# jacobwulffwold/GAN_SR_wind_field

Hardware: AMD Instinct MI355X
Metric: GAN train-steps/sec (G+D fwd+bwd) (higher is better)
Workload: dtype bf16; 1 GPU; C3' full G+D adversarial step: LR 32x32x128 -> HR 128x128x128 (x4), batch 1/GPU, G 16 RRDB nf128 (34.77M), D bf32; preset=C3p, global_batch=1, parallelism=dp1, ranks=1

## Files before the change

### gan_sr_wind_field_amd/csrc/conv_tile.hip

```cpp
#include <cstdlib>

#include "conv_tile_impl.h"

int wsr_ct_run_n144(CtArgs& a, int tpk, hipStream_t st);
int wsr_ct_run_n128(CtArgs& a, int tpk, hipStream_t st);
int wsr_ct_run_narrow(CtArgs& a, int tpk, hipStream_t st);
int wsr_ct_run_wide(CtArgs& a, int tpk, hipStream_t st);
int wsr_ct_run_masked(CtArgs& a, int tpk, hipStream_t st);
int wsr_ct_run_narrow_masked(CtArgs& a, int tpk, hipStream_t st);
int wsr_ct_run_small(CtArgs& a, int tpk, hipStream_t st);
int wsr_ct_run_tm3(CtArgs& a, int tpk, hipStream_t st);
int wsr_ct_run_simple_narrow(CtArgs& a, int tpk, int tm3, hipStream_t st);
int wsr_ct_run_simple_n128(CtArgs& a, int tpk, int tm3, hipStream_t st);
int wsr_ct_run_simple_small(CtArgs& a, int tpk, hipStream_t st);
long wsr_ct_tiles(const CtArgs& a, int rows);
int wsr_ct_run_strided(CtArgs& a, int tpk, hipStream_t st);
int wsr_ct_run_f32(CtArgs& a, int tpk, hipStream_t st);

namespace {

int dispatch_ct(CtArgs& a, int tpk, hipStream_t st) {
  const int N = a.Cout;
  if (a.f32) return wsr_ct_run_f32(a, tpk, st);
  if ((a.sx | a.sy | a.sz) != 1) return wsr_ct_run_strided(a, tpk, st);
// ... 450 lines not shown
  a.alpha = 1.f;
  if (ep) {
    a.bias = ep->bias;
    a.chan_scale = ep->chan_scale;
    a.res = (const unsigned short*)ep->res;
    a.res_ctot = ep->res_ctot;
    a.res_off = ep->res_off;
    a.res_c1 = 0x7FFFFFFF;
    a.alpha = ep->alpha;
    a.beta = ep->beta;
    a.slope = ep->slope;
    a.act = ep->act;
    a.act_c1 = ep->act_c1 > 0 ? ep->act_c1 : 0x7FFFFFFF;
    if (a.act == 2 && (!a.res || ep->out_planar)) return WSR_EINVAL;
    a.out_planar = ep->out_planar;
    if (a.res && (a.res_off < 0 || a.res_off + c->Cout > a.res_ctot)) return WSR_EINVAL;
    a.ws = ep->ws;
    a.ws_bytes = (long)ep->ws_bytes;
    if (two) {
      a.in2 = (const unsigned short*)ep->in2;
      a.in2_ctot = ep->in2_ctot;
      a.in2_chunk = ep->in2_c0;
    }
    if (ep->mask) {
      const wsr_lrelu_mask_t* mk = ep->mask;
      if (!mk->y || ep->out_planar || mk->c0 < 0 || mk->c1 > c->Cout || mk->c0 >= mk->c1 || mk->c0 % 4 || mk->y_ctot % 4 ||
          mk->y_off % 4 || mk->y_off + (mk->c1 - mk->c0) > mk->y_ctot || mk->chan_scale)
        return WSR_EINVAL;
      if (f32) return WSR_EUNSUPPORTED;
      a.mask_y = (const unsigned short*)mk->y;
      a.mask_ctot = mk->y_ctot; a.mask_off = mk->y_off;
      a.mask_c0 = mk->c0; a.mask_c1 = mk->c1;
      a.mask_slope = mk->slope;
    }
  }
  a.B = c->B; a.Xi = c->Xi; a.Yi = c->Yi; a.Zi = c->Zi;
  a.Xo = c->Xo; a.Yo = c->Yo; a.Zo = c->Zo;
  a.ups = c->upsample_xy ? 1 : 0;
  a.in_ctot = c->in_ctot; a.in_off = c->in_off;
  a.Cout = c->Cout; a.out_ctot = c->out_ctot; a.out_off = c->out_off;
  a.KX = c->KX; a.KY = c->KY; a.KZ = c->KZ;
  a.px = c->px; a.py = c->py; a.pz = c->pz;
  if (c->lat) {
    if (a.res || a.out_planar) return WSR_EUNSUPPORTED;
    a.ol_m = 2; a.ol_ox = c->lat_ox; a.ol_oy = c->lat_oy;
    a.ol_mz = c->lat_mz > 1 ? c->lat_mz : 1; a.ol_oz = c->lat_oz;
    a.nphase = c->lat_phases == 4 ? 4 : 1;
    a.ph_wstride = (long)wsr_frag_filter_elems(c->Cout, c->Cin, c->KX * c->KY * c->KZ, c->dtype);
  }
  if (f32 && c->KX * c->KY * c->KZ == 1) return WSR_EUNSUPPORTED;
  if (!f32 && !a.mask_y && c->KX * c->KY * c->KZ == 1 && !c->lat && !a.ups && !a.out_planar && !a.chan_scale && (c->px | c->py | c->pz) == 0 &&
      (c->sx | c->sy | c->sz) == 1 && a.act <= 1 && a.act_c1 == 0x7FFFFFFF) {
    const int rc = wsr_conv1x1_bf16(a.in, a.in_ctot, a.in_off, c->Cin, a.wf, (unsigned short*)a.out, a.out_ctot,
                                    a.out_off, a.Cout, (long)c->B * c->Xo * c->Yo * c->Zo, a.bias, a.res, a.res_ctot,
                                    a.res_off, a.res ? a.res_c1 : 0, a.alpha, a.beta, a.act, a.slope, nullptr,
                                    ep ? (const unsigned short*)ep->res2 : nullptr, ep ? ep->res2_ctot : 0,
                                    ep ? ep->res2_off : 0, ep ? ep->beta2 : 0.f, as_stream(stream));
    if (rc != WSR_EUNSUPPORTED) return rc;
  }
  if (ep && ep->res2) return WSR_EUNSUPPORTED;
  if (two) return run_conv_tile(a, c->Cin, as_stream(stream));
  const bool no_slide = WSR_ENV_SET("WSR_NO_SLIDE");
  if (!f32 && !no_slide && c->KZ == 1 && c->Cout <= 16 && a.out_planar && !a.chan_scale && !a.res && a.act == 0 && !a.ups &&
      !c->lat && (c->sx | c->sy | c->sz) == 1 && c->pz == 0 && a.alpha == 1.f && c->Xo == c->Xi && c->Yo == c->Yi &&
      zero_page()) {
    const int rc = wsr_conv_slide_fwd(a.in, a.in_ctot, a.in_off, c->Cin, a.wf, (float*)a.out, c->Cout, c->B, c->Xi, c->Yi,
// ... 107 lines not shown
```

### gan_sr_wind_field_amd/csrc/conv_tile_impl.h

```cpp
#pragma once
#include <cstdlib>
#include <type_traits>

#include "common.h"

struct CtArgs {
  const unsigned short* in;
  const unsigned short* wf;
  void* out;
  const void* zero16;
  const float* bias;
  const float* chan_scale;
  const unsigned short* res;
  int res_ctot, res_off, res_c1;
  float alpha, beta, slope;
  int act, out_planar;
  int act_c1;
  int B, Xi, Yi, Zi, Xo, Yo, Zo, ups;
  int in_ctot, in_off, nchunks;
  int cin_valid;
  int Cout, out_ctot, out_off;
  int KX, KY, KZ, px, py, pz;
  int sx, sy, sz;
  int TX, TY, TZ;
  int tiles_x, tiles_y, tiles_z, ntiles;
  int nts;
  int TS;
  int NT_total;
  int ngroups;
  int P;
  int off_mtab, off_htab, off_ttab, off_btab, off_xs, off_ws;
  int vec_ok;
  const unsigned short* mask_y;
  int mask_ctot, mask_off, mask_c0, mask_c1;
  float mask_slope;
  int xbufs;
  unsigned mg_TZ, mg_TY, mg_Lz, mg_Ly, mg_KZ, mg_KY, mg_ng, mg_tz, mg_ty, mg_tx;
  int il_m, il_ox, il_oy, ol_m, ol_ox, ol_oy, nphase;
  int ol_mz, ol_oz;
  long ph_wstride;
  int ksplit, cps;
  float* part;
  long part_stride;
  void* ws;
  long ws_bytes;
  int xs_stage, xs_units;
  const unsigned short* in2;
  int in2_ctot, in2_chunk;
  void* out2;
  int out2_ctot, out2_c0;
  int f32;
  int prio;
  int ablate;
  unsigned long long* stamps;
};

int wsr_ct_splitk_reduce(const CtArgs& a, hipStream_t st);

void wsr_ct_note_plan(const CtArgs& a, int ntw);
void wsr_ct_note_inst(int wm, int wn, int tm, int tn, int tpk, int mask, int f32, int wk, int simple);

namespace {

__device__ __forceinline__ void glds16(const void* gsrc, unsigned lds_addr) {
  unsigned keep;
  asm volatile(
      "s_mov_b32 %0, m0\n\ts_mov_b32 m0, %2\n\ts_nop 0\n\tglobal_load_lds_dwordx4 %1, off\n\ts_mov_b32 m0, %0"
      : "=&s"(keep)
      : "v"(gsrc), "s"(lds_addr)
      : "memory");
}
__device__ __forceinline__ void dma_wait() { asm volatile("s_waitcnt vmcnt(0)" ::: "memory"); }

#ifdef WSR_CT_STAMPS
#define CT_STAMP(k)                                                                                   \
  do {                                                                                                \
    if (a.stamps && threadIdx.x == 0) a.stamps[(size_t)blockIdx.x * 8 + (k)] = (k) >= 6 ? clock64() : wall_clock64(); \
  } while (0)
#else
#define CT_STAMP(k) do {} while (0)
#endif

__device__ __forceinline__ unsigned fdiv(unsigned n, unsigned d, unsigned mg) { return d == 1 ? n : __umulhi(n, mg); }
static inline unsigned fdiv_magic(int d) { return d <= 1 ? 0u : (unsigned)(((1ull << 32) + d - 1) / d); }

constexpr bool ct_two_src(int wn, int tn) { return wn == 1 && tn == 9; }
constexpr int ct_xk(int waves, int tm) { return waves <= 4 ? 16 : (tm <= 2 ? 13 : 10); }
// ... 451 lines not shown
#pragma unroll
    for (int i = 0; i < TM; ++i) {
      if (mrow[i] < 0) continue;
      float v[4];
      const bool act_here = a.act && co0 < a.act_c1;
      if (fast && a.act == 2) {
        const float4 rv = ct_cvt4<T>(rr[s][i]);
        const float r4[4] = {rv.x, rv.y, rv.z, rv.w};
#pragma unroll
        for (int q = 0; q < 4; ++q) {
          float x = acc[i][j][q] + bb[s][q] + a.beta * r4[q];
          if (act_here) x = x > 0.f ? x : x * a.slope;
          v[q] = x * ss[s][q];
        }
        st4<T>(orow[i] + 16 * j, make_float4(v[0], v[1], v[2], v[3]));
        continue;
      }
#pragma unroll
      for (int q = 0; q < 4; ++q) {
        float x = acc[i][j][q] + bb[s][q];
        if (act_here) x = x > 0.f ? x : x * a.slope;
        v[q] = x * ss[s][q];
      }
      if (fast) {
        float4 o4 = make_float4(v[0], v[1], v[2], v[3]);
        if (a.res) {
          const float4 rv = ct_cvt4<T>(rr[s][i]);
          o4.x += a.beta * rv.x;
          o4.y += a.beta * rv.y;
          o4.z += a.beta * rv.z;
          o4.w += a.beta * rv.w;
        }
        if constexpr (MASK) {
          const float4 mk = ct_mask4<T>(yy[s][i], a.mask_slope);
          o4.x *= mk.x;
          o4.y *= mk.y;
          o4.z *= mk.z;
          o4.w *= mk.w;
        }
#ifdef WSR_CT_STAMPS
        if constexpr (sizeof(E) == 2) {
          if (a.ablate & 32) {
            if (!(j & 1) && j + 1 < TN) {
              float4 d4 = o4;
              d4.x += acc[i][j + 1][0];
              d4.y += acc[i][j + 1][1];
              union { uint4 u; unsigned short h[8]; } pk;
              pk.h[0] = f2bf(o4.x); pk.h[1] = f2bf(o4.y); pk.h[2] = f2bf(o4.z); pk.h[3] = f2bf(o4.w);
              pk.h[4] = f2bf(d4.x); pk.h[5] = f2bf(d4.y); pk.h[6] = f2bf(d4.z); pk.h[7] = f2bf(d4.w);
              *reinterpret_cast<uint4*>(orow[i] + 16 * j + 4 * fg) = pk.u;
              continue;
            }
            if ((j & 1)) continue;
          }
        }
#endif
        if constexpr (TWO) {
          if (a.out2 && co0 >= a.out2_c0) {
            st4<T>(reinterpret_cast<E*>(a.out2) + mrow[i] * a.out2_ctot + (co0 - a.out2_c0), o4);
            continue;
          }
        }
        st4<T>(orow[i] + 16 * j, o4);
        continue;
      }
      const long vi = mrow[i] - (long)b * vox_per_b;
#pragma unroll
      for (int q = 0; q < 4; ++q) {
        if (co0 + q >= a.Cout) continue;
        float x = v[q];
        if (out_planar) {
          reinterpret_cast<float*>(a.out)[((long)b * a.Cout + co0 + q) * vox_per_b + vi] = x;
        } else {
          if (a.res && co0 + q < a.res_c1)
            x += a.beta * ldf<T>(reinterpret_cast<const E*>(a.res) + mrow[i] * a.res_ctot + a.res_off + co0 + q);
          if constexpr (MASK) {
            if (co0 + q >= a.mask_c0 && co0 + q < a.mask_c1)
              x *= ldf<T>(reinterpret_cast<const E*>(a.mask_y) + mrow[i] * a.mask_ctot + a.mask_off + (co0 + q - a.mask_c0)) > 0.f
                       ? 1.f : a.mask_slope;
          }
          stf<T>(reinterpret_cast<E*>(a.out) + mrow[i] * a.out_ctot + a.out_off + co0 + q, x);
        }
      }
    }
  }
  CT_STAMP(5);
  CT_STAMP(7);
#ifdef WSR_CT_STAMPS
  if (a.stamps && lane == 0 && (wave == 0 || wave == WAVES - 1)) {
    unsigned long long* p = a.stamps + ((size_t)gridDim.x + 2 * blockIdx.x + (wave ? 1 : 0)) * 8;
    p[0] = (unsigned long long)st_dma;
    p[1] = (unsigned long long)st_bar;
    p[2] = (unsigned long long)total_phases;
  }
#endif
}

static inline int round_up(int v, int m) { return (v + m - 1) / m * m; }

template <int WM, int WN, int TM, int TN, int TPK, bool MASK = false, class T = BF16, int WK = 1, int SIMPLE = 0>
int launch_ct(CtArgs& a, hipStream_t st) {
  constexpr int WAVES = WM * WN * WK, NTW = WN * TN;
  const int taps = a.KX * a.KY * a.KZ;
  constexpr int M = WM * TM * 16;
  if (a.TX * a.TY * a.TZ > M) return WSR_EUNSUPPORTED;
  if (a.in2 || a.out2) {
    constexpr int CKH = T::EPP * (4 / TPK);
    if (!ct_two_src(WN, TN) || a.ups || a.nphase == 4) return WSR_EUNSUPPORTED;
    if (a.in2 && (a.in2_ctot % T::EPP || a.in2_chunk < 1 || a.in2_chunk * CKH >= a.cin_valid)) return WSR_EINVAL;
// ... 175 lines not shown
```

### gan_sr_wind_field_amd/csrc/physics_loss.hip

```cpp
#include "common.h"
#include "stencil.h"

namespace {

constexpr int PL_BLOCK = 256;
constexpr int PL_ROWS = 1024;
constexpr int PL_NS = 6, PL_NM = 8, PL_N = PL_NS + PL_NM;

__device__ __forceinline__ float nanmax(float m, float v) { return (m != m || v != v) ? __builtin_nanf("") : fmaxf(m, v); }

struct Jac { float j[9]; };
__device__ __forceinline__ Jac jacobian(const float* __restrict__ p, long vol, long plane, int Z, int x, int y, int z, int X,
                                        int Y, const Row3& wx, const Row3& wy, const Row3& wz) {
  Jac o;
#pragma unroll
  for (int c = 0; c < 3; ++c) {
    const float* fp = p + (long)c * vol;
    const float f0 = *fp;
    o.j[c] = (x > 0 ? wx.a * fp[-plane] : 0.f) + wx.b * f0 + (x < X - 1 ? wx.c * fp[plane] : 0.f);
    o.j[3 + c] = (y > 0 ? wy.a * fp[-Z] : 0.f) + wy.b * f0 + (y < Y - 1 ? wy.c * fp[Z] : 0.f);
    o.j[6 + c] = (z > 0 ? wz.a * fp[-1] : 0.f) + wz.b * f0 + (z < Z - 1 ? wz.c * fp[1] : 0.f);
  }
  return o;
}

__global__ __launch_bounds__(PL_BLOCK) void physics_stats_kernel(const float* __restrict__ hr, const float* __restrict__ sr,
                                                                const float* __restrict__ xs, const float* __restrict__ ys,
                                                                const float* __restrict__ zc, float* __restrict__ part, int B,
                                                                int X, int Y, int Z) {
  const long plane = (long)Y * Z, vol = (long)X * plane, total = (long)B * vol;
  float s[PL_NS] = {0.f, 0.f, 0.f, 0.f, 0.f, 0.f};
  const float ninf = -__builtin_inff();
  float m[PL_NM] = {0.f, ninf, 0.f, 0.f, 0.f, ninf, 0.f, 0.f};
  for (long i = blockIdx.x * (long)blockDim.x + threadIdx.x; i < total; i += (long)gridDim.x * blockDim.x) {
    const int z = (int)(i % Z);
    long r = i / Z;
    const int y = (int)(r % Y); r /= Y;
    const int x = (int)(r % X);
    const long b = r / X;
    const long sp = (long)x * plane + (long)y * Z + z;
    const Row3 wx = deriv_row(Lin{xs, 1}, x, X), wy = deriv_row(Lin{ys, 1}, y, Y);
    const Row3 wz = deriv_row(Lin{zc + b * vol + (long)x * plane + (long)y * Z, 1}, z, Z);
    const float* hp = hr + b * 3 * vol + sp;
    const float* qp = sr + b * 3 * vol + sp;
    const Jac jh = jacobian(hp, vol, plane, Z, x, y, z, X, Y, wx, wy, wz);
    const Jac js = jacobian(qp, vol, plane, Z, x, y, z, X, Y, wx, wy, wz);
#pragma unroll
    for (int c = 0; c < 9; ++c) {
      const float d = js.j[c] - jh.j[c];
      if (c < 6) {
        s[0] += d * d;
        m[0] = nanmax(m[0], fabsf(jh.j[c]));
        m[4] = nanmax(m[4], fabsf(js.j[c]));
      } else {
        s[1] += d * d;
        m[1] = nanmax(m[1], jh.j[c]);
        m[5] = nanmax(m[5], js.j[c]);
      }
    }
    const float h2 = jh.j[0] + jh.j[4], s2 = js.j[0] + js.j[4];
    const float h3 = h2 + jh.j[8], s3 = s2 + js.j[8];
    s[2] += (h3 - s3) * (h3 - s3);
    s[3] += (h2 - s2) * (h2 - s2);
    m[2] = nanmax(m[2], fabsf(h3)); m[6] = nanmax(m[6], fabsf(s3));
    m[3] = nanmax(m[3], fabsf(h2)); m[7] = nanmax(m[7], fabsf(s2));
#pragma unroll
    for (int c = 0; c < 3; ++c) {
      const float d = hp[(long)c * vol] - qp[(long)c * vol];
      s[4] += fabsf(d);
      s[5] += d * d;
    }
  }
#pragma unroll
  for (int off = 32; off > 0; off >>= 1) {
#pragma unroll
    for (int k = 0; k < PL_NS; ++k) s[k] += __shfl_xor(s[k], off, 64);
#pragma unroll
    for (int k = 0; k < PL_NM; ++k) m[k] = nanmax(m[k], __shfl_xor(m[k], off, 64));
  }
  __shared__ float sh[PL_BLOCK / 64][PL_N];
  const int wave = threadIdx.x >> 6, lane = threadIdx.x & 63;
  if (lane == 0) {
#pragma unroll
    for (int k = 0; k < PL_NS; ++k) sh[wave][k] = s[k];
#pragma unroll
    for (int k = 0; k < PL_NM; ++k) sh[wave][PL_NS + k] = m[k];
  }
  __syncthreads();
  if (threadIdx.x < PL_N) {
    const int k = threadIdx.x;
    float a = sh[0][k];
    for (int w = 1; w < PL_BLOCK / 64; ++w) a = k < PL_NS ? a + sh[w][k] : nanmax(a, sh[w][k]);
    part[(long)blockIdx.x * PL_N + k] = a;
  }
}

__global__ __launch_bounds__(64 * PL_N) void physics_stats_final_kernel(const float* __restrict__ part, int rows,
                                                                       float* __restrict__ out) {
  const int k = threadIdx.x >> 6, lane = threadIdx.x & 63;
  if (k < PL_NS) {
    double a = 0.0;
    for (int r = lane; r < rows; r += 64) a += (double)part[(long)r * PL_N + k];
#pragma unroll
    for (int off = 32; off > 0; off >>= 1) a += __shfl_xor(a, off, 64);
    if (lane == 0) out[k] = (float)a;
  } else {
    float a = part[k];
    for (int r = lane; r < rows; r += 64) a = nanmax(a, part[(long)r * PL_N + k]);
#pragma unroll
    for (int off = 32; off > 0; off >>= 1) a = nanmax(a, __shfl_xor(a, off, 64));
    if (lane == 0) out[k] = a;
  }
}

__global__ __launch_bounds__(PL_BLOCK) void physics_residual_kernel(const float* __restrict__ hr, const float* __restrict__ sr,
                                                                   const float* __restrict__ xs, const float* __restrict__ ys,
                                                                   const float* __restrict__ zc, const float* __restrict__ coef,
                                                                   float* __restrict__ res, int B, int X, int Y, int Z) {
  const long plane = (long)Y * Z, vol = (long)X * plane, total = (long)B * vol;
  const float g0 = 2.f * coef[0], g1 = 2.f * coef[1], g2 = 2.f * coef[2], g3 = 2.f * coef[3];
  const bool on0 = g0 != 0.f, on1 = g1 != 0.f, on2 = g2 != 0.f, on3 = g3 != 0.f;
  for (long i = blockIdx.x * (long)blockDim.x + threadIdx.x; i < total; i += (long)gridDim.x * blockDim.x) {
    const int z = (int)(i % Z);
    long r = i / Z;
    const int y = (int)(r % Y); r /= Y;
    const int x = (int)(r % X);
    const long b = r / X;
    const long sp = (long)x * plane + (long)y * Z + z;
    const Row3 wx = deriv_row(Lin{xs, 1}, x, X), wy = deriv_row(Lin{ys, 1}, y, Y);
    const Row3 wz = deriv_row(Lin{zc + b * vol + (long)x * plane + (long)y * Z, 1}, z, Z);
    const Jac jh = jacobian(hr + b * 3 * vol + sp, vol, plane, Z, x, y, z, X, Y, wx, wy, wz);
    const Jac js = jacobian(sr + b * 3 * vol + sp, vol, plane, Z, x, y, z, X, Y, wx, wy, wz);
    float o[9];
#pragma unroll
    for (int c = 0; c < 9; ++c) o[c] = (c < 6 ? on0 : on1) ? (c < 6 ? g0 : g1) * (js.j[c] - jh.j[c]) : 0.f;
    const float d2 = (js.j[0] + js.j[4]) - (jh.j[0] + jh.j[4]);
    const float d3 = d2 + (js.j[8] - jh.j[8]);
    const float t3 = on2 ? g2 * d3 : 0.f;
    const float t = t3 + (on3 ? g3 * d2 : 0.f);
    o[0] += t; o[4] += t; o[8] += t3;
    float* rp = res + b * 9 * vol + sp;
#pragma unroll
    for (int c = 0; c < 9; ++c) rp[(long)c * vol] = o[c];
  }
}

// ... 13 lines not shown
    const int c = (int)(r % 3);
    const long b = r / 3;
    const long gb = ((b * 9) * vol) + (long)x * plane + (long)y * Z + z;
    float acc = 0.f;
    if (phys) {
    {
      const float* gp = res + gb + (long)(0 + c) * vol;
      const Lin co{xs, 1};
      acc += deriv_row(co, x, X).b * gp[0];
      if (x > 0) acc += deriv_row(co, x - 1, X).c * gp[-plane];
      if (x < X - 1) acc += deriv_row(co, x + 1, X).a * gp[plane];
    }
    {
      const float* gp = res + gb + (long)(3 + c) * vol;
      const Lin co{ys, 1};
      acc += deriv_row(co, y, Y).b * gp[0];
      if (y > 0) acc += deriv_row(co, y - 1, Y).c * gp[-Z];
      if (y < Y - 1) acc += deriv_row(co, y + 1, Y).a * gp[Z];
    }
    {
      const float* gp = res + gb + (long)(6 + c) * vol;
      const Lin co{zc + (b * vol + (long)x * plane + (long)y * Z), 1};
      acc += deriv_row(co, z, Z).b * gp[0];
      if (z > 0) acc += deriv_row(co, z - 1, Z).c * gp[-1];
      if (z < Z - 1) acc += deriv_row(co, z + 1, Z).a * gp[1];
    }
    }
    const float d = sr[i] - hr[i];
    acc += (c1 != 0.f ? c1 * (d > 0.f ? 1.f : (d < 0.f ? -1.f : 0.f)) : 0.f) + (c2 != 0.f ? c2 * d : 0.f);
    dsr[i] = acc;
  }
}

inline int pl_grid(long n) {
  long g = (n + PL_BLOCK - 1) / PL_BLOCK;
  if (g > PL_ROWS) g = PL_ROWS;
  return g < 1 ? 1 : (int)g;
}

}

extern "C" int64_t wsr_physics_loss_workspace_floats(void) { return (int64_t)PL_ROWS * PL_N; }

extern "C" int wsr_physics_loss_stats(const float* hr, const float* sr, const float* xs, const float* ys, const float* zc,
                                      float* stats, float* workspace, int32_t B, int32_t X, int32_t Y, int32_t Z,
                                      void* stream) {
  if (!hr || !sr || !xs || !ys || !zc || !stats || !workspace || B <= 0 || X <= 0 || Y <= 0 || Z <= 0) return WSR_EINVAL;
  const int grid = pl_grid((long)B * X * Y * Z);
  hipLaunchKernelGGL(physics_stats_kernel, dim3(grid), dim3(PL_BLOCK), 0, as_stream(stream), hr, sr, xs, ys, zc, workspace,
                     B, X, Y, Z);
  WSR_LAUNCH_CHECK();
  hipLaunchKernelGGL(physics_stats_final_kernel, dim3(1), dim3(64 * PL_N), 0, as_stream(stream), workspace, grid, stats);
  WSR_LAUNCH_CHECK();
  return 0;
}

extern "C" int wsr_physics_loss_bwd(const float* hr, const float* sr, const float* xs, const float* ys, const float* zc,
                                    const float* coef, float* residual, float* dsr, int32_t B, int32_t X, int32_t Y,
                                    int32_t Z, void* stream) {
  if (!hr || !sr || !xs || !ys || !zc || !coef || !residual || !dsr || B <= 0 || X <= 0 || Y <= 0 || Z <= 0)
    return WSR_EINVAL;
  const long nvox = (long)B * X * Y * Z;
  long g = (nvox + PL_BLOCK - 1) / PL_BLOCK;
  if (g > 65535 * 16) g = 65535 * 16;
  hipLaunchKernelGGL(physics_residual_kernel, dim3((unsigned)g), dim3(PL_BLOCK), 0, as_stream(stream), hr, sr, xs, ys, zc,
                     coef, residual, B, X, Y, Z);
  WSR_LAUNCH_CHECK();
  long g3 = (3 * nvox + PL_BLOCK - 1) / PL_BLOCK;
  if (g3 > 65535 * 16) g3 = 65535 * 16;
  hipLaunchKernelGGL(physics_adjoint_kernel, dim3((unsigned)g3), dim3(PL_BLOCK), 0, as_stream(stream), residual, hr, sr,
                     xs, ys, zc, coef, dsr, B, X, Y, Z);
  WSR_LAUNCH_CHECK();
  return 0;
}
```

### gan_sr_wind_field_amd/csrc/stencil.h

```cpp
#pragma once
#include "common.h"

namespace {

struct Row3 { float a, b, c; };
template <class Coord>
__device__ __forceinline__ Row3 deriv_row(const Coord& co, int i, int n) {
  Row3 r;
  if (n < 2) { r.a = r.b = r.c = 0.f; return r; }
  if (i == 0) { const float h = co(1) - co(0); r.a = 0.f; r.b = -1.f / h; r.c = 1.f / h; return r; }
  if (i == n - 1) { const float h = co(n - 1) - co(n - 2); r.a = -1.f / h; r.b = 1.f / h; r.c = 0.f; return r; }
  const float hl = co(i) - co(i - 1), hr = co(i + 1) - co(i);
  const float den = hl * hr * (hl + hr);
  r.a = -(hr * hr) / den; r.b = (hr * hr - hl * hl) / den; r.c = (hl * hl) / den;
  return r;
}
struct Lin { const float* p; long s; __device__ float operator()(int i) const { return p[(long)i * s]; } };

}
```

### gan_sr_wind_field_amd/engine.py

```python
from __future__ import annotations

from dataclasses import dataclass
from typing import Callable, Dict, List, Optional, Sequence, Tuple

import torch
from torch import nn

from . import hip_ops as ops
from .hip_ops import ConvGeom

Tensor = torch.Tensor

STACK_DGRAD = __import__("os").environ.get("WSR_STACK_DGRAD", "1") != "0"
STACK_FWD = __import__("os").environ.get("WSR_STACK_FWD", "1") != "0"
FUSED_BN_STATS = __import__("os").environ.get("WSR_FUSED_BN_STATS", "1") != "0"
GD_INPLACE = __import__("os").environ.get("WSR_GD_INPLACE", "1") != "0"
GD_PINGPONG = __import__("os").environ.get("WSR_GD_PINGPONG", "1") != "0"
ZFOLD = __import__("os").environ.get("WSR_ZFOLD", "1") != "0"
WGRAD_STREAM = int(__import__("os").environ.get("WSR_WGRAD_STREAM", "0"))
F32_TILE = __import__("os").environ.get("WSR_F32_TILE", "1") != "0"
SWAP_THIN_WGRAD = __import__("os").environ.get("WSR_THIN_WGRAD_SWAP", "1") != "0"
SPLIT_CAT = __import__("os").environ.get("WSR_SPLIT_CAT", "1") != "0"
POISON_BUFFERS = bool(int(__import__("os").environ.get("WSR_POISON_BUFFERS", "0")))
DETERMINISTIC = __import__("os").environ.get("WSR_DETERMINISTIC", "1") != "0"
ARENA_MB = int(__import__("os").environ.get("WSR_ARENA_MB", "1024"))
STRIDED_DGRAD = __import__("os").environ.get("WSR_STRIDED_DGRAD", "1") != "0"
STRIDED_WGRAD = __import__("os").environ.get("WSR_STRIDED_WGRAD", "1") != "0"
SUBPIXEL = __import__("os").environ.get("WSR_SUBPIXEL", "1") != "0"
SUBPIXEL_WGRAD = __import__("os").environ.get("WSR_SUBPIXEL_WGRAD", "1") != "0"
WGRAD_LAT4 = __import__("os").environ.get("WSR_WGRAD_LAT4", "1") != "0"
LFF_BIAS_FUSED = __import__("os").environ.get("WSR_LFF_BIAS_FUSED", "1") != "0"


def compute_dtype_of(flag) -> torch.dtype:
    if isinstance(flag, torch.dtype):
        return flag
    if isinstance(flag, str):
        return {"fp32": torch.float32, "f32": torch.float32, "bf16": torch.bfloat16}[flag.lower()]
    return torch.bfloat16 if flag else torch.float32


class FilterCache:

    def __init__(self, frag_dt: torch.dtype = torch.bfloat16):
        self._c: Dict[tuple, tuple] = {}
        self._tables: Dict[tuple, tuple] = {}
        self._gen = 0
        self.frag_dt = frag_dt

    def get(self, p: Tensor, dt: torch.dtype, transpose: bool, kpad: int, rows_pad: int) -> Tensor:
        key = (id(p), dt, transpose, kpad, rows_pad)
        stamp = (p._version, p.data_ptr(), p.device, self._gen)
        hit = self._c.get(key)
        if hit is not None and hit[0] == stamp:
            return hit[1]
        w = p.detach()
        if w.dim() == 2:
            raise ValueError("filters are 5-D")
        w = w.contiguous()
# ... 1405 lines not shown
        return True

    def conv_sites(self) -> Sequence[ConvSite]:
        sites = list(self.all_sites)
        for li, groups in self.dparity.items():
            if self.strided_dgrad_active(li):
                for _, _, par in groups:
                    sites += par
        return sites

    def refresh_filters(self, backward: bool) -> None:
        if backward:
            for li, groups in self.dparity.items():
                if not self.strided_dgrad_active(li):
                    continue
                w = self.layers[li].conv.weight
                fresh = False
                for g in groups:
                    zc, wp, par = g
                    if wp.device != w.device:
                        wp = g[1] = torch.empty_like(wp, device=w.device)
                        for ph, s in enumerate(par):
                            s.weight = wp[ph]
                        fresh = True
                    fresh = self._seed_parity_frags(par, w.device) or fresh
                stamp = (w._version, w.data_ptr(), self.filters._gen)
                if fresh or stamp != self._dparity_stamp.get(li):
                    for zc, wp, par in groups:
                        ops.strided_parity_filters(w.detach().contiguous(), wp, self.layers[li].conv.stride[2], zc)
                    self.filters.touch()
                    self._dparity_stamp[li] = stamp
        super().refresh_filters(backward)

    def strided_dgrad(self, li: int, gy: Tensor, gin: Tensor) -> None:
        s = self.layers[li].conv
        sz = s.stride[2]
        B, oxyz = gy.shape[0], tuple(gy.shape[1:4])

        def run():
            for zc, wp, par in self.dparity[li]:
                frs, batched = self._parity_frags(par)
                g = ConvGeom(s.cout, s.cin, par[0].kernel, (1, 1, 1), par[0].pad)
                if batched:
                    d = ops.make_desc(g, self.dt, B, oxyz, gy.shape[-1], 0, gin.shape[-1], 0, cin=self.cp(s.cout),
                                      cout=self.cp(s.cin), lat=(0, 0, 4, sz, zc))
                    if ops.conv_fwd_tile(d, gy, frs[0], gin):
                        continue
                for ph, ps in enumerate(par):
                    d = ops.make_desc(ConvGeom(s.cout, s.cin, ps.kernel, (1, 1, 1), ps.pad), self.dt, B, oxyz,
                                      gy.shape[-1], 0, gin.shape[-1], 0, cin=self.cp(s.cout), cout=self.cp(s.cin),
                                      lat=(ph >> 1, ph & 1, 0, sz, zc))
                    if not ops.conv_fwd_tile(d, gy, frs[ph], gin):
                        raise RuntimeError("strided input gradient outside the tile kernels (set WSR_STRIDED_DGRAD=0)")

        if self.launch_probe is not None:
            self.launch_probe("dgrad:" + s.name, run)
        else:
            run()

    def forward(self, x, training: bool, save: bool):
        sl = self.slope
        xs = tuple(x) if isinstance(x, (tuple, list)) else (x,)
        G, Bg = len(xs), xs[0].shape[0]
        B = G * Bg
        ops._need_cuda(*xs, self.layers[0].conv.weight)
        self.refresh_filters(backward=save)
        c0 = self.cp(self.layers[0].conv.cin)
        h = self._empty((B,) + tuple(xs[0].shape[2:]) + (c0,), xs[0])
        for gi, xg in enumerate(xs):
            if xg.shape != xs[0].shape:
                raise ValueError("grouped discriminator inputs must have one shape")
            ops.planar_to_ndhwc(xg.contiguous().float(), h[gi * Bg:(gi + 1) * Bg], 0, c0)
        x = xs[0]
        recs = []
        nbt: Dict[int, list] = {}
        eval_consts: Dict[int, tuple] = {}
        if not training:
            bns = [l.bn for l in self.layers if l.bn is not None and not l.inorm]
            if bns:
                with torch.no_grad():
                    inv = torch._foreach_add([b.running_var.detach().float() for b in bns], [b.eps for b in bns]) \
                        if len({b.eps for b in bns}) > 1 else torch._foreach_add([b.running_var.detach().float() for b in bns], bns[0].eps)
                    torch._foreach_rsqrt_(inv)
                eval_consts = {id(b): (b.running_mean.detach().float(), v) for b, v in zip(bns, inv)}
        for l in self.layers:
            s = l.conv
            g = ConvGeom(s.cin, s.cout, s.kernel, s.stride, s.pad)
            oxyz = g.out_extent(*h.shape[1:4])
            cp_out = self.cp(s.cout)
            y = self._empty((B,) + oxyz + (cp_out,), x, zero=cp_out != s.cout)
            if l.bn is None:
# ... 91 lines not shown
            with torch.no_grad():
                for calls in sorted({c for _, c in nbt.values()}):
                    torch._foreach_add_([t for t, c in nbt.values() if c == calls], calls)
        saved = dict(recs=recs, in_shape=tuple(x.shape), groups=G, group_batch=Bg) if save else None
        return h, saved

    def backward(self, saved: dict, g_feat: Tensor, need_dx: bool, need_dw: bool, lo: int = 0):
        sl = self.slope
        dev = g_feat.device
        flat = self.space.new(dev) if need_dw else None
        scratch = None
        if need_dw:
            self.begin_backward(dev)
        sp = self.space
        done = 0
        Bg = saved.get("group_batch", g_feat.shape[0])
        if lo and (need_dw or lo % Bg):
            raise ValueError("a partial backward pass starts at a group boundary and has no parameter gradients")
        g = g_feat.contiguous()
        dx = None
        recs = saved["recs"]
        bn_grad_jobs: Dict[int, tuple] = {}

        def flush_bn_grads():
            with torch.no_grad():
                for gi in sorted(bn_grad_jobs):
                    dst, src = bn_grad_jobs[gi]
                    if gi == 0:
                        torch._foreach_copy_(dst, src)
                    else:
                        torch._foreach_add_(dst, src)
            bn_grad_jobs.clear()

        for li in reversed(range(len(self.layers))):
            l, r = self.layers[li], recs[li]
            s = l.conv
            C_ = s.cout
            act_o = r["a"][lo:]
            if self.trace is not None:
                self.trace.append(("g", li, g.clone()))
            if l.bn is None:
                if l.act:
                    ops.lrelu_bwd_(g, 0, act_o, 0, g.shape[-1], sl)
                gy = g
            else:
                bn = l.bn
                y_o = r["y"][lo:]
                gy = self._empty(y_o.shape, g)
                if r.get("inorm"):
                    one, _ = self._unit(C_, dev)
                    for b in range(g.shape[0]):
                        sums = torch.empty(2 * C_, dtype=torch.float32, device=dev)
                        ops.bn_bwd_reduce(g[b:b + 1], act_o[b:b + 1], y_o[b:b + 1], r["mean"][lo + b], r["invstd"][lo + b],
                                          l.act, sl, sums)
                        ops.bn_bwd_apply(g[b:b + 1], y_o[b:b + 1], gy[b:b + 1], r["mean"][lo + b], r["invstd"][lo + b], one,
                                         sums, 1.0 / r["count"][lo + b])
                elif r["training"]:
                    G = r["groups"]
                    g0 = lo // Bg
                    sums_all = torch.empty((G - g0, 2 * C_), dtype=torch.float32, device=dev)
                    for gi in range(g0, G):
                        o = gi * Bg - lo
                        gg, ag, yg = g[o:o + Bg], act_o[o:o + Bg], y_o[o:o + Bg]
                        sums = sums_all[gi - g0]
                        ops.bn_bwd_reduce(gg, ag, yg, r["mean"][gi], r["invstd"][gi], l.act, sl, sums)
                        if need_dw:
                            bn_dst = [sp.view(flat, bn.bias), sp.view(flat, bn.weight)]
                            bn_grad_jobs.setdefault(gi, ([], []))
                            bn_grad_jobs[gi][0].extend(bn_dst)
                            bn_grad_jobs[gi][1].extend([sums[:C_], sums[C_:]])
                    if self.stat_allreduce is not None:
                        sums_all = sums_all.clone()
                        self.stat_allreduce(sums_all)
                    for gi in range(g0, G):
                        o = gi * Bg - lo
                        gg, yg, gyg = g[o:o + Bg], y_o[o:o + Bg], gy[o:o + Bg]
                        ops.bn_bwd_apply(gg, yg, gyg, r["mean"][gi], r["invstd"][gi], bn.weight.detach(),
                                         sums_all[gi - g0], 1.0 / r["count"][gi])
                else:
                    mean, invstd = r["mean"][0], r["invstd"][0]
                    fused = (l.act and not need_dw and
                             ops.bn_bwd_apply(g, y_o, gy, mean, invstd, bn.weight.detach(), None, 0.0, act_y=act_o, slope=sl))
                    if not fused:
                        if l.act:
                            ops.lrelu_bwd_(g, 0, act_o, 0, g.shape[-1], sl)
                        if need_dw:
                            sums = torch.empty(2 * C_, dtype=torch.float32, device=dev)
                            ops.bn_bwd_reduce(g, act_o, y_o, mean, invstd, False, sl, sums)
                            sp.view(flat, bn.bias).copy_(sums[:C_])
                            sp.view(flat, bn.weight).copy_(sums[C_:])
                        ops.bn_bwd_apply(g, y_o, gy, mean, invstd, bn.weight.detach(), None, 0.0)
            if self.trace is not None:
                self.trace.append(("gy", li, gy.clone()))
            inp = r["inp"][lo:]
            lattice_ok = (li in self.dparity and tuple(inp.shape[1:3]) == (2 * gy.shape[1], 2 * gy.shape[2])
                          and inp.shape[3] == s.stride[2] * gy.shape[3] and inp.shape[-1] == self.cp(s.cin))
            if need_dw:
                if not (lattice_ok and self.strided_wgrad_active(li) and self.strided_wgrad(li, inp, gy, flat, sp)):
                    self.wgrad(s, inp, 0, gy, 0, flat, sp, scratch)
                if self.grad_ready_hook is not None:
                    flush_bn_grads()
                    hi = sp.offsets[id(s.weight)][0] + (s.weight.numel() + 63) // 64 * 64
                    self.grad_ready_hook(flat, done, hi, self.flush_unpack)
                    done = hi
            if li > 0:
                gin = self._empty(inp.shape, g)
                if self.strided_dgrad_active(li) and lattice_ok:
                    self.strided_dgrad(li, gy, gin)
                else:
                    self.dgrad(s, gy, 0, gin, 0, tuple(inp.shape[1:4]))
                if self.trace is not None:
                    self.trace.append(("gin", li, gin.clone()))
                g = gin
            elif need_dx:
                dx = torch.empty((inp.shape[0],) + tuple(saved["in_shape"][1:]), dtype=torch.float32, device=dev)
                self.dgrad(s, gy, 0, dx, 0, tuple(inp.shape[1:4]), dx_planar=True)
        if need_dw:
            flush_bn_grads()
            self.end_backward()
        if need_dw and self.grad_done_hook is not None:
            self.grad_done_hook()
        return dx, flat


class _DiscriminatorFeaturesFn(torch.autograd.Function):
    @staticmethod
    def forward(ctx, x, prog: DiscriminatorProgram, training: bool, save: bool, *params):
        feat, saved = prog.forward(x, training, save)
        ctx.prog, ctx.saved = prog, saved
        ctx.feat_c = prog.layers[-1].conv.cout
        return feat[..., :ctx.feat_c].permute(0, 4, 1, 2, 3).float()

    @staticmethod
    def backward(ctx, g_out):
        prog, saved = ctx.prog, ctx.saved
        if saved is None:
            raise RuntimeError("Discriminator_3D.features backward without saved activations")
        need_dx = ctx.needs_input_grad[0]
        need_dw = any(ctx.needs_input_grad[4:])
        c = ctx.feat_c
        cp_ = prog.cp(c)
# ... 64 lines not shown
```

Before: 11.22 train-steps/s.

## Fold LeakyReLU backward mask into strided dgrad epilogue and preload physics stencil

The discriminator's strided (lattice) input-gradient convolutions can now take the layer-below activation as a LeakyReLU mask and apply it in the conv epilogue, so the separate lrelu_bwd pass over the gradient is skipped. To keep numerics consistent with the unfused path, the output is rounded to bf16 before masking. A fallback records shapes where the masked tile path fails and reruns unmasked. Separately, the physics stats kernel gains a variant that preloads all stencil neighbours and coordinate values into registers before computing the Jacobians.

```diff
diff --git a/gan_sr_wind_field_amd/csrc/conv_tile.hip b/gan_sr_wind_field_amd/csrc/conv_tile.hip
--- a/gan_sr_wind_field_amd/csrc/conv_tile.hip
+++ b/gan_sr_wind_field_amd/csrc/conv_tile.hip
@@ -506,6 +506,7 @@
       a.mask_ctot = mk->y_ctot; a.mask_off = mk->y_off;
       a.mask_c0 = mk->c0; a.mask_c1 = mk->c1;
       a.mask_slope = mk->slope;
+      a.mask_round = c->lat ? 1 : 0;
     }
   }
   a.B = c->B; a.Xi = c->Xi; a.Yi = c->Yi; a.Zi = c->Zi;
diff --git a/gan_sr_wind_field_amd/csrc/conv_tile_impl.h b/gan_sr_wind_field_amd/csrc/conv_tile_impl.h
--- a/gan_sr_wind_field_amd/csrc/conv_tile_impl.h
+++ b/gan_sr_wind_field_amd/csrc/conv_tile_impl.h
@@ -53,6 +53,7 @@
   int prio;
   int ablate;
   unsigned long long* stamps;
+  int mask_round;
 };
 
 int wsr_ct_splitk_reduce(const CtArgs& a, hipStream_t st);
@@ -570,6 +571,9 @@
           o4.w += a.beta * rv.w;
         }
         if constexpr (MASK) {
+          if constexpr (!SIMPLE && sizeof(E) == 2) {
+            if (a.mask_round) o4 = make_float4(bf2f(f2bf(o4.x)), bf2f(f2bf(o4.y)), bf2f(f2bf(o4.z)), bf2f(f2bf(o4.w)));
+          }
           const float4 mk = ct_mask4<T>(yy[s][i], a.mask_slope);
           o4.x *= mk.x;
           o4.y *= mk.y;
@@ -613,6 +617,9 @@
           if (a.res && co0 + q < a.res_c1)
             x += a.beta * ldf<T>(reinterpret_cast<const E*>(a.res) + mrow[i] * a.res_ctot + a.res_off + co0 + q);
           if constexpr (MASK) {
+            if constexpr (!SIMPLE && sizeof(E) == 2) {
+              if (a.mask_round) x = bf2f(f2bf(x));
+            }
             if (co0 + q >= a.mask_c0 && co0 + q < a.mask_c1)
               x *= ldf<T>(reinterpret_cast<const E*>(a.mask_y) + mrow[i] * a.mask_ctot + a.mask_off + (co0 + q - a.mask_c0)) > 0.f
                        ? 1.f : a.mask_slope;
diff --git a/gan_sr_wind_field_amd/csrc/physics_loss.hip b/gan_sr_wind_field_amd/csrc/physics_loss.hip
--- a/gan_sr_wind_field_amd/csrc/physics_loss.hip
+++ b/gan_sr_wind_field_amd/csrc/physics_loss.hip
@@ -1,117 +1,8 @@
 #include "common.h"
 #include "stencil.h"
+#include "physics_stats_kernels.h"
 
 namespace {
-
-constexpr int PL_BLOCK = 256;
-constexpr int PL_ROWS = 1024;
-constexpr int PL_NS = 6, PL_NM = 8, PL_N = PL_NS + PL_NM;
-
-__device__ __forceinline__ float nanmax(float m, float v) { return (m != m || v != v) ? __builtin_nanf("") : fmaxf(m, v); }
-
-struct Jac { float j[9]; };
-__device__ __forceinline__ Jac jacobian(const float* __restrict__ p, long vol, long plane, int Z, int x, int y, int z, int X,
-                                        int Y, const Row3& wx, const Row3& wy, const Row3& wz) {
-  Jac o;
-#pragma unroll
-  for (int c = 0; c < 3; ++c) {
-    const float* fp = p + (long)c * vol;
-    const float f0 = *fp;
-    o.j[c] = (x > 0 ? wx.a * fp[-plane] : 0.f) + wx.b * f0 + (x < X - 1 ? wx.c * fp[plane] : 0.f);
-    o.j[3 + c] = (y > 0 ? wy.a * fp[-Z] : 0.f) + wy.b * f0 + (y < Y - 1 ? wy.c * fp[Z] : 0.f);
-    o.j[6 + c] = (z > 0 ? wz.a * fp[-1] : 0.f) + wz.b * f0 + (z < Z - 1 ? wz.c * fp[1] : 0.f);
-  }
-  return o;
-}
-
-__global__ __launch_bounds__(PL_BLOCK) void physics_stats_kernel(const float* __restrict__ hr, const float* __restrict__ sr,
-                                                                const float* __restrict__ xs, const float* __restrict__ ys,
-                                                                const float* __restrict__ zc, float* __restrict__ part, int B,
-                                                                int X, int Y, int Z) {
-  const long plane = (long)Y * Z, vol = (long)X * plane, total = (long)B * vol;
-  float s[PL_NS] = {0.f, 0.f, 0.f, 0.f, 0.f, 0.f};
-  const float ninf = -__builtin_inff();
-  float m[PL_NM] = {0.f, ninf, 0.f, 0.f, 0.f, ninf, 0.f, 0.f};
-  for (long i = blockIdx.x * (long)blockDim.x + threadIdx.x; i < total; i += (long)gridDim.x * blockDim.x) {
-    const int z = (int)(i % Z);
-    long r = i / Z;
-    const int y = (int)(r % Y); r /= Y;
-    const int x = (int)(r % X);
-    const long b = r / X;
-    const long sp = (long)x * plane + (long)y * Z + z;
-    const Row3 wx = deriv_row(Lin{xs, 1}, x, X), wy = deriv_row(Lin{ys, 1}, y, Y);
-    const Row3 wz = deriv_row(Lin{zc + b * vol + (long)x * plane + (long)y * Z, 1}, z, Z);
-    const float* hp = hr + b * 3 * vol + sp;
-    const float* qp = sr + b * 3 * vol + sp;
-    const Jac jh = jacobian(hp, vol, plane, Z, x, y, z, X, Y, wx, wy, wz);
-    const Jac js = jacobian(qp, vol, plane, Z, x, y, z, X, Y, wx, wy, wz);
-#pragma unroll
-    for (int c = 0; c < 9; ++c) {
-      const float d = js.j[c] - jh.j[c];
-      if (c < 6) {
-        s[0] += d * d;
-        m[0] = nanmax(m[0], fabsf(jh.j[c]));
-        m[4] = nanmax(m[4], fabsf(js.j[c]));
-      } else {
-        s[1] += d * d;
-        m[1] = nanmax(m[1], jh.j[c]);
-        m[5] = nanmax(m[5], js.j[c]);
-      }
-    }
-    const float h2 = jh.j[0] + jh.j[4], s2 = js.j[0] + js.j[4];
-    const float h3 = h2 + jh.j[8], s3 = s2 + js.j[8];
-    s[2] += (h3 - s3) * (h3 - s3);
-    s[3] += (h2 - s2) * (h2 - s2);
-    m[2] = nanmax(m[2], fabsf(h3)); m[6] = nanmax(m[6], fabsf(s3));
-    m[3] = nanmax(m[3], fabsf(h2)); m[7] = nanmax(m[7], fabsf(s2));
-#pragma unroll
-    for (int c = 0; c < 3; ++c) {
-      const float d = hp[(long)c * vol] - qp[(long)c * vol];
-      s[4] += fabsf(d);
-      s[5] += d * d;
-    }
-  }
-#pragma unroll
-  for (int off = 32; off > 0; off >>= 1) {
-#pragma unroll
-    for (int k = 0; k < PL_NS; ++k) s[k] += __shfl_xor(s[k], off, 64);
-#pragma unroll
-    for (int k = 0; k < PL_NM; ++k) m[k] = nanmax(m[k], __shfl_xor(m[k], off, 64));
-  }
-  __shared__ float sh[PL_BLOCK / 64][PL_N];
-  const int wave = threadIdx.x >> 6, lane = threadIdx.x & 63;
-  if (lane == 0) {
-#pragma unroll
-    for (int k = 0; k < PL_NS; ++k) sh[wave][k] = s[k];
-#pragma unroll
-    for (int k = 0; k < PL_NM; ++k) sh[wave][PL_NS + k] = m[k];
-  }
-  __syncthreads();
-  if (threadIdx.x < PL_N) {
-    const int k = threadIdx.x;
-    float a = sh[0][k];
-    for (int w = 1; w < PL_BLOCK / 64; ++w) a = k < PL_NS ? a + sh[w][k] : nanmax(a, sh[w][k]);
-    part[(long)blockIdx.x * PL_N + k] = a;
-  }
-}
-
-__global__ __launch_bounds__(64 * PL_N) void physics_stats_final_kernel(const float* __restrict__ part, int rows,
-                                                                       float* __restrict__ out) {
-  const int k = threadIdx.x >> 6, lane = threadIdx.x & 63;
-  if (k < PL_NS) {
-    double a = 0.0;
-    for (int r = lane; r < rows; r += 64) a += (double)part[(long)r * PL_N + k];
-#pragma unroll
-    for (int off = 32; off > 0; off >>= 1) a += __shfl_xor(a, off, 64);
-    if (lane == 0) out[k] = (float)a;
-  } else {
-    float a = part[k];
-    for (int r = lane; r < rows; r += 64) a = nanmax(a, part[(long)r * PL_N + k]);
-#pragma unroll
-    for (int off = 32; off > 0; off >>= 1) a = nanmax(a, __shfl_xor(a, off, 64));
-    if (lane == 0) out[k] = a;
-  }
-}
 
 __global__ __launch_bounds__(PL_BLOCK) void physics_residual_kernel(const float* __restrict__ hr, const float* __restrict__ sr,
                                                                    const float* __restrict__ xs, const float* __restrict__ ys,
@@ -191,12 +82,6 @@
   }
 }
 
-inline int pl_grid(long n) {
-  long g = (n + PL_BLOCK - 1) / PL_BLOCK;
-  if (g > PL_ROWS) g = PL_ROWS;
-  return g < 1 ? 1 : (int)g;
-}
-
 }
 
 extern "C" int64_t wsr_physics_loss_workspace_floats(void) { return (int64_t)PL_ROWS * PL_N; }
@@ -206,8 +91,12 @@
                                       void* stream) {
   if (!hr || !sr || !xs || !ys || !zc || !stats || !workspace || B <= 0 || X <= 0 || Y <= 0 || Z <= 0) return WSR_EINVAL;
   const int grid = pl_grid((long)B * X * Y * Z);
-  hipLaunchKernelGGL(physics_stats_kernel, dim3(grid), dim3(PL_BLOCK), 0, as_stream(stream), hr, sr, xs, ys, zc, workspace,
-                     B, X, Y, Z);
+  if (WSR_ENV_INT("WSR_PHYSICS_STATS_PRELOAD", 1))
+    hipLaunchKernelGGL(physics_stats_preload_kernel, dim3(grid), dim3(PL_BLOCK), 0, as_stream(stream), hr, sr, xs, ys, zc,
+                       workspace, B, X, Y, Z);
+  else
+    hipLaunchKernelGGL(physics_stats_kernel, dim3(grid), dim3(PL_BLOCK), 0, as_stream(stream), hr, sr, xs, ys, zc, workspace,
+                       B, X, Y, Z);
   WSR_LAUNCH_CHECK();
   hipLaunchKernelGGL(physics_stats_final_kernel, dim3(1), dim3(64 * PL_N), 0, as_stream(stream), workspace, grid, stats);
   WSR_LAUNCH_CHECK();
diff --git a/gan_sr_wind_field_amd/csrc/physics_stats_kernels.h b/gan_sr_wind_field_amd/csrc/physics_stats_kernels.h
--- /dev/null
+++ b/gan_sr_wind_field_amd/csrc/physics_stats_kernels.h
@@ -0,0 +1,228 @@
+#pragma once
+#include "stencil.h"
+
+namespace {
+
+constexpr int PL_BLOCK = 256;
+constexpr int PL_ROWS = 1024;
+constexpr int PL_NS = 6, PL_NM = 8, PL_N = PL_NS + PL_NM;
+
+__device__ __forceinline__ float nanmax(float m, float v) { return (m != m || v != v) ? __builtin_nanf("") : fmaxf(m, v); }
+
+struct Jac { float j[9]; };
+__device__ __forceinline__ Jac jacobian(const float* __restrict__ p, long vol, long plane, int Z, int x, int y, int z, int X,
+                                        int Y, const Row3& wx, const Row3& wy, const Row3& wz) {
+  Jac o;
+#pragma unroll
+  for (int c = 0; c < 3; ++c) {
+    const float* fp = p + (long)c * vol;
+    const float f0 = *fp;
+    o.j[c] = (x > 0 ? wx.a * fp[-plane] : 0.f) + wx.b * f0 + (x < X - 1 ? wx.c * fp[plane] : 0.f);
+    o.j[3 + c] = (y > 0 ? wy.a * fp[-Z] : 0.f) + wy.b * f0 + (y < Y - 1 ? wy.c * fp[Z] : 0.f);
+    o.j[6 + c] = (z > 0 ? wz.a * fp[-1] : 0.f) + wz.b * f0 + (z < Z - 1 ? wz.c * fp[1] : 0.f);
+  }
+  return o;
+}
+
+__global__ __launch_bounds__(PL_BLOCK) void physics_stats_kernel(const float* __restrict__ hr, const float* __restrict__ sr,
+                                                                const float* __restrict__ xs, const float* __restrict__ ys,
+                                                                const float* __restrict__ zc, float* __restrict__ part, int B,
+                                                                int X, int Y, int Z) {
+  const long plane = (long)Y * Z, vol = (long)X * plane, total = (long)B * vol;
+  float s[PL_NS] = {0.f, 0.f, 0.f, 0.f, 0.f, 0.f};
+  const float ninf = -__builtin_inff();
+  float m[PL_NM] = {0.f, ninf, 0.f, 0.f, 0.f, ninf, 0.f, 0.f};
+  for (long i = blockIdx.x * (long)blockDim.x + threadIdx.x; i < total; i += (long)gridDim.x * blockDim.x) {
+    const int z = (int)(i % Z);
+    long r = i / Z;
+    const int y = (int)(r % Y); r /= Y;
+    const int x = (int)(r % X);
+    const long b = r / X;
+    const long sp = (long)x * plane + (long)y * Z + z;
+    const Row3 wx = deriv_row(Lin{xs, 1}, x, X), wy = deriv_row(Lin{ys, 1}, y, Y);
+    const Row3 wz = deriv_row(Lin{zc + b * vol + (long)x * plane + (long)y * Z, 1}, z, Z);
+    const float* hp = hr + b * 3 * vol + sp;
+    const float* qp = sr + b * 3 * vol + sp;
+    const Jac jh = jacobian(hp, vol, plane, Z, x, y, z, X, Y, wx, wy, wz);
+    const Jac js = jacobian(qp, vol, plane, Z, x, y, z, X, Y, wx, wy, wz);
+#pragma unroll
+    for (int c = 0; c < 9; ++c) {
+      const float d = js.j[c] - jh.j[c];
+      if (c < 6) {
+        s[0] += d * d;
+        m[0] = nanmax(m[0], fabsf(jh.j[c]));
+        m[4] = nanmax(m[4], fabsf(js.j[c]));
+      } else {
+        s[1] += d * d;
+        m[1] = nanmax(m[1], jh.j[c]);
+        m[5] = nanmax(m[5], js.j[c]);
+      }
+    }
+    const float h2 = jh.j[0] + jh.j[4], s2 = js.j[0] + js.j[4];
+    const float h3 = h2 + jh.j[8], s3 = s2 + js.j[8];
+    s[2] += (h3 - s3) * (h3 - s3);
+    s[3] += (h2 - s2) * (h2 - s2);
+    m[2] = nanmax(m[2], fabsf(h3)); m[6] = nanmax(m[6], fabsf(s3));
+    m[3] = nanmax(m[3], fabsf(h2)); m[7] = nanmax(m[7], fabsf(s2));
+#pragma unroll
+    for (int c = 0; c < 3; ++c) {
+      const float d = hp[(long)c * vol] - qp[(long)c * vol];
+      s[4] += fabsf(d);
+      s[5] += d * d;
+    }
+  }
+#pragma unroll
+  for (int off = 32; off > 0; off >>= 1) {
+#pragma unroll
+    for (int k = 0; k < PL_NS; ++k) s[k] += __shfl_xor(s[k], off, 64);
+#pragma unroll
+    for (int k = 0; k < PL_NM; ++k) m[k] = nanmax(m[k], __shfl_xor(m[k], off, 64));
+  }
+  __shared__ float sh[PL_BLOCK / 64][PL_N];
+  const int wave = threadIdx.x >> 6, lane = threadIdx.x & 63;
+  if (lane == 0) {
+#pragma unroll
+    for (int k = 0; k < PL_NS; ++k) sh[wave][k] = s[k];
+#pragma unroll
+    for (int k = 0; k < PL_NM; ++k) sh[wave][PL_NS + k] = m[k];
+  }
+  __syncthreads();
+  if (threadIdx.x < PL_N) {
+    const int k = threadIdx.x;
+    float a = sh[0][k];
+    for (int w = 1; w < PL_BLOCK / 64; ++w) a = k < PL_NS ? a + sh[w][k] : nanmax(a, sh[w][k]);
+    part[(long)blockIdx.x * PL_N + k] = a;
+  }
+}
+
+struct Pre3 {
+  float cm, c0, cp;
+  int i;
+  __device__ __forceinline__ float operator()(int k) const { return k < i ? cm : (k > i ? cp : c0); }
+};
+
+__device__ __forceinline__ Jac jacobian_vals(const float (&f)[3][7], int x, int y, int z, int X, int Y, int Z, const Row3& wx,
+                                             const Row3& wy, const Row3& wz) {
+  Jac o;
+#pragma unroll
+  for (int c = 0; c < 3; ++c) {
+    const float f0 = f[c][0];
+    o.j[c] = (x > 0 ? wx.a * f[c][1] : 0.f) + wx.b * f0 + (x < X - 1 ? wx.c * f[c][2] : 0.f);
+    o.j[3 + c] = (y > 0 ? wy.a * f[c][3] : 0.f) + wy.b * f0 + (y < Y - 1 ? wy.c * f[c][4] : 0.f);
+    o.j[6 + c] = (z > 0 ? wz.a * f[c][5] : 0.f) + wz.b * f0 + (z < Z - 1 ? wz.c * f[c][6] : 0.f);
+  }
+  return o;
+}
+
+__global__ __launch_bounds__(PL_BLOCK) void physics_stats_preload_kernel(const float* __restrict__ hr,
+                                                                        const float* __restrict__ sr,
+                                                                        const float* __restrict__ xs,
+                                                                        const float* __restrict__ ys,
+                                                                        const float* __restrict__ zc, float* __restrict__ part,
+                                                                        int B, int X, int Y, int Z) {
+  const long plane = (long)Y * Z, vol = (long)X * plane, total = (long)B * vol;
+  float s[PL_NS] = {0.f, 0.f, 0.f, 0.f, 0.f, 0.f};
+  const float ninf = -__builtin_inff();
+  float m[PL_NM] = {0.f, ninf, 0.f, 0.f, 0.f, ninf, 0.f, 0.f};
+  for (long i = blockIdx.x * (long)blockDim.x + threadIdx.x; i < total; i += (long)gridDim.x * blockDim.x) {
+    const int z = (int)(i % Z);
+    long r = i / Z;
+    const int y = (int)(r % Y); r /= Y;
+    const int x = (int)(r % X);
+    const long b = r / X;
+    const long sp = (long)x * plane + (long)y * Z + z;
+    const long off[7] = {0, x > 0 ? -plane : 0, x < X - 1 ? plane : 0, y > 0 ? -(long)Z : 0, y < Y - 1 ? (long)Z : 0,
+                         z > 0 ? -1L : 0, z < Z - 1 ? 1L : 0};
+    const float* hp = hr + b * 3 * vol + sp;
+    const float* qp = sr + b * 3 * vol + sp;
+    const float* zp = zc + b * vol + sp;
+    float h[3][7], q[3][7];
+#pragma unroll
+    for (int c = 0; c < 3; ++c)
+#pragma unroll
+      for (int k = 0; k < 7; ++k) {
+        h[c][k] = hp[(long)c * vol + off[k]];
+        q[c][k] = qp[(long)c * vol + off[k]];
+      }
+    const Pre3 cz{zp[off[5]], zp[0], zp[off[6]], z};
+    const Pre3 cx{xs[x > 0 ? x - 1 : 0], xs[x], xs[x < X - 1 ? x + 1 : x], x};
+    const Pre3 cy{ys[y > 0 ? y - 1 : 0], ys[y], ys[y < Y - 1 ? y + 1 : y], y};
+    const Row3 wx = deriv_row(cx, x, X), wy = deriv_row(cy, y, Y);
+    const Row3 wz = deriv_row(cz, z, Z);
+    const Jac jh = jacobian_vals(h, x, y, z, X, Y, Z, wx, wy, wz);
+    const Jac js = jacobian_vals(q, x, y, z, X, Y, Z, wx, wy, wz);
+#pragma unroll
+    for (int c = 0; c < 9; ++c) {
+      const float d = js.j[c] - jh.j[c];
+      if (c < 6) {
+        s[0] += d * d;
+        m[0] = nanmax(m[0], fabsf(jh.j[c]));
+        m[4] = nanmax(m[4], fabsf(js.j[c]));
+      } else {
+        s[1] += d * d;
+        m[1] = nanmax(m[1], jh.j[c]);
+        m[5] = nanmax(m[5], js.j[c]);
+      }
+    }
+    const float h2 = jh.j[0] + jh.j[4], s2 = js.j[0] + js.j[4];
+    const float h3 = h2 + jh.j[8], s3 = s2 + js.j[8];
+    s[2] += (h3 - s3) * (h3 - s3);
+    s[3] += (h2 - s2) * (h2 - s2);
+    m[2] = nanmax(m[2], fabsf(h3)); m[6] = nanmax(m[6], fabsf(s3));
+    m[3] = nanmax(m[3], fabsf(h2)); m[7] = nanmax(m[7], fabsf(s2));
+#pragma unroll
+    for (int c = 0; c < 3; ++c) {
+      const float d = h[c][0] - q[c][0];
+      s[4] += fabsf(d);
+      s[5] += d * d;
+    }
+  }
+#pragma unroll
+  for (int off = 32; off > 0; off >>= 1) {
+#pragma unroll
+    for (int k = 0; k < PL_NS; ++k) s[k] += __shfl_xor(s[k], off, 64);
+#pragma unroll
+    for (int k = 0; k < PL_NM; ++k) m[k] = nanmax(m[k], __shfl_xor(m[k], off, 64));
+  }
+  __shared__ float sh[PL_BLOCK / 64][PL_N];
+  const int wave = threadIdx.x >> 6, lane = threadIdx.x & 63;
+  if (lane == 0) {
+#pragma unroll
+    for (int k = 0; k < PL_NS; ++k) sh[wave][k] = s[k];
+#pragma unroll
+    for (int k = 0; k < PL_NM; ++k) sh[wave][PL_NS + k] = m[k];
+  }
+  __syncthreads();
+  if (threadIdx.x < PL_N) {
+    const int k = threadIdx.x;
+    float a = sh[0][k];
+    for (int w = 1; w < PL_BLOCK / 64; ++w) a = k < PL_NS ? a + sh[w][k] : nanmax(a, sh[w][k]);
+    part[(long)blockIdx.x * PL_N + k] = a;
+  }
+}
+
+__global__ __launch_bounds__(64 * PL_N) void physics_stats_final_kernel(const float* __restrict__ part, int rows,
+                                                                       float* __restrict__ out) {
+  const int k = threadIdx.x >> 6, lane = threadIdx.x & 63;
+  if (k < PL_NS) {
+    double a = 0.0;
+    for (int r = lane; r < rows; r += 64) a += (double)part[(long)r * PL_N + k];
+#pragma unroll
+    for (int off = 32; off > 0; off >>= 1) a += __shfl_xor(a, off, 64);
+    if (lane == 0) out[k] = (float)a;
+  } else {
+    float a = part[k];
+    for (int r = lane; r < rows; r += 64) a = nanmax(a, part[(long)r * PL_N + k]);
+#pragma unroll
+    for (int off = 32; off > 0; off >>= 1) a = nanmax(a, __shfl_xor(a, off, 64));
+    if (lane == 0) out[k] = a;
+  }
+}
+
+inline int pl_grid(long n) {
+  long g = (n + PL_BLOCK - 1) / PL_BLOCK;
+  if (g > PL_ROWS) g = PL_ROWS;
+  return g < 1 ? 1 : (int)g;
+}
+
+}
diff --git a/gan_sr_wind_field_amd/csrc/stencil.h b/gan_sr_wind_field_amd/csrc/stencil.h
--- a/gan_sr_wind_field_amd/csrc/stencil.h
+++ b/gan_sr_wind_field_amd/csrc/stencil.h
@@ -1,5 +1,7 @@
 #pragma once
+#ifndef WSR_HOST_CHECK
 #include "common.h"
+#endif
 
 namespace {
 
diff --git a/gan_sr_wind_field_amd/engine.py b/gan_sr_wind_field_amd/engine.py
--- a/gan_sr_wind_field_amd/engine.py
+++ b/gan_sr_wind_field_amd/engine.py
@@ -25,6 +25,7 @@
 DETERMINISTIC = __import__("os").environ.get("WSR_DETERMINISTIC", "1") != "0"
 ARENA_MB = int(__import__("os").environ.get("WSR_ARENA_MB", "1024"))
 STRIDED_DGRAD = __import__("os").environ.get("WSR_STRIDED_DGRAD", "1") != "0"
+STRIDED_DGRAD_MASK = __import__("os").environ.get("WSR_STRIDED_DGRAD_MASK", "1") != "0"
 STRIDED_WGRAD = __import__("os").environ.get("WSR_STRIDED_WGRAD", "1") != "0"
 SUBPIXEL = __import__("os").environ.get("WSR_SUBPIXEL", "1") != "0"
 SUBPIXEL_WGRAD = __import__("os").environ.get("WSR_SUBPIXEL_WGRAD", "1") != "0"
@@ -1496,31 +1497,48 @@
                     self._dparity_stamp[li] = stamp
         super().refresh_filters(backward)
 
-    def strided_dgrad(self, li: int, gy: Tensor, gin: Tensor) -> None:
+    def strided_dgrad(self, li: int, gy: Tensor, gin: Tensor, mask: Optional[Tensor] = None) -> bool:
         s = self.layers[li].conv
         sz = s.stride[2]
         B, oxyz = gy.shape[0], tuple(gy.shape[1:4])
-
-        def run():
+        bad_key = ("dmask", li, B) + oxyz
+        m = None
+        if mask is not None and bad_key not in self._dparity_bad:
+            m = (mask, 0, 0, self.cp(s.cin), self.slope)
+        masked = [False]
+
+        def launches(m) -> bool:
             for zc, wp, par in self.dparity[li]:
                 frs, batched = self._parity_frags(par)
                 g = ConvGeom(s.cout, s.cin, par[0].kernel, (1, 1, 1), par[0].pad)
                 if batched:
                     d = ops.make_desc(g, self.dt, B, oxyz, gy.shape[-1], 0, gin.shape[-1], 0, cin=self.cp(s.cout),
                                       cout=self.cp(s.cin), lat=(0, 0, 4, sz, zc))
-                    if ops.conv_fwd_tile(d, gy, frs[0], gin):
+                    if ops.conv_fwd_tile(d, gy, frs[0], gin, mask=m):
                         continue
                 for ph, ps in enumerate(par):
                     d = ops.make_desc(ConvGeom(s.cout, s.cin, ps.kernel, (1, 1, 1), ps.pad), self.dt, B, oxyz,
                                       gy.shape[-1], 0, gin.shape[-1], 0, cin=self.cp(s.cout), cout=self.cp(s.cin),
                                       lat=(ph >> 1, ph & 1, 0, sz, zc))
-                    if not ops.conv_fwd_tile(d, gy, frs[ph], gin):
+                    if not ops.conv_fwd_tile(d, gy, frs[ph], gin, mask=m):
+                        if m is not None:
+                            return False
                         raise RuntimeError("strided input gradient outside the tile kernels (set WSR_STRIDED_DGRAD=0)")
+            return True
+
+        def run():
+            if m is not None:
+                if launches(m):
+                    masked[0] = True
+                    return
+                self._dparity_bad.add(bad_key)
+            launches(None)
 
         if self.launch_probe is not None:
             self.launch_probe("dgrad:" + s.name, run)
         else:
             run()
+        return masked[0]
 
     def forward(self, x, training: bool, save: bool):
         sl = self.slope
@@ -1678,6 +1696,7 @@
                         torch._foreach_add_(dst, src)
             bn_grad_jobs.clear()
 
+        g_masked = False
         for li in reversed(range(len(self.layers))):
             l, r = self.layers[li], recs[li]
             s = l.conv
@@ -1686,7 +1705,7 @@
             if self.trace is not None:
                 self.trace.append(("g", li, g.clone()))
             if l.bn is None:
-                if l.act:
+                if l.act and not g_masked:
                     ops.lrelu_bwd_(g, 0, act_o, 0, g.shape[-1], sl)
                 gy = g
             else:
@@ -1751,8 +1770,11 @@
                     done = hi
             if li > 0:
                 gin = self._empty(inp.shape, g)
+                g_masked = False
                 if self.strided_dgrad_active(li) and lattice_ok:
-                    self.strided_dgrad(li, gy, gin)
+                    below = self.layers[li - 1]
+                    fold = STRIDED_DGRAD_MASK and below.bn is None and bool(below.act) and self.trace is None
+                    g_masked = self.strided_dgrad(li, gy, gin, mask=inp if fold else None)
                 else:
                     self.dgrad(s, gy, 0, gin, 0, tuple(inp.shape[1:4]))
                 if self.trace is not None:
```

Result: no change. 11.25 train-steps/s, median of 2 (+0.3%).
